# swarth100/dynfu

Measured on AMD Instinct MI355X. Metric: frames/sec (warp-solve + TSDF fuse), 512^3 vol / 2k nodes / VGA depth, higher is better.
Workload: dtype f32; 1 GPU; C2: 512^3 TSDF, 640x480 depth, 2048 nodes, k=4, 262144 vertices, 5 GN x PCG<=256 (tol 1e-6), reference-parity energy (energy.t), lambda=200; parallelism=replicas x1 (one sequence per GPU, no collective), ranks_seen=1, repeats=5

## Files before the change

dynfu_amd/csrc/capi_solver.cpp:

```cpp
#include <algorithm>
#include <cmath>
#include <cstdlib>
#include <cstring>
#include <new>

#include "capi_internal.hpp"
#include "dev_switch.hpp"
#include "solve.hpp"

using namespace dfa::capi;

struct dfa_solver {
    int max_D, max_N, k;
    size_t max_R;
    int ell_cap;
    int asm_resident = 0;
    dfa::SolveView v;
    dfa::SolveState* state;
    double* cost_partials;
    unsigned int* ticket;
    dfa::PlanArena mem;
    GridScratch grid;
    bool has_problem;
    bool timing;
// ... 92 lines not shown
        const size_t areas = (size_t)3 * dfa::solve_team_pcg_rounds();
        mem.alloc(&s->v.team_ctl, 1, true);
        mem.alloc(&s->v.team_mt, areas * s->v.team_stride, true);
        mem.alloc(&s->v.team_words, dfa::solve_team_pcg_words(), true);
        s->team.host_abort = mem.pinned<int>(1);
        if ((rc = plan_status(mem)) == DFA_OK && !s->team.host_abort) rc = fail(DFA_ERR_HIP, "hipHostMalloc (team PCG abort count)");
        if (rc == DFA_OK) {
            s->team.ctl = s->v.team_ctl;
            if (const char* e0 = dfa::dev_env("DFA_MB_TEAM_EPOCH")) s->team.epoch = (unsigned)std::strtoul(e0, nullptr, 0);
        }
    }
    if (rc == DFA_OK) {
        mem.alloc(&s->state, 1);
        mem.alloc(&s->iters_total, 1, true);
        s->host_flag = mem.pinned<int>(4);
        mem.alloc(&s->cost_partials, std::max<size_t>((R + 255) / 256 + 1, 1024) + 1024);
        mem.alloc(&s->ticket, 64, true);
        rc = plan_status(mem);
    }
    if (rc != DFA_OK) {
        dfa_solver_destroy(s);
        return rc;
    }
    *out = s;
    return DFA_OK;
}

void dfa_solver_destroy(dfa_solver* s) {
    if (!s) return;
    s->grid.release();
    s->mb_graphs.release();
// ... 84 lines not shown
                HIP_TRY(hipMemcpyAsync(&s->host_flag[1], &s->state->converged, sizeof(int), hipMemcpyDeviceToHost, st));
                HIP_TRY(hipStreamSynchronize(st));
            }
            if (s->host_flag && s->host_flag[1]) {
                ++not_launched;
                continue;
            }
            ++gn_in_outer;
            if (gn > 0 && p->gn_tol == 0.f && p->lambda > 0.f && !no_regradient) {
                const int ev = bracket_open(s, st);
                HIP_TRY(dfa::solve_regradient(v, s->state, st));
                if (int rc = run_pcg(ev)) return rc;
                continue;
            }
            const bool with_huber = gn == 0 && outer == p->num_iter - 1;
            HIP_TRY(dfa::solve_linearise(v, s->state, s->cost_partials, s->ticket, gn == 0, gn == 0 ? 0 : 1,
                                         p->gn_tol, p->tukey_offset, p->psi_data, w_reg_sq, with_huber ? p->psi_reg : 0.f, nullptr, st));
            huber_done |= with_huber;
            const int ev = bracket_open(s, st);
            HIP_TRY(dfa::solve_assemble(v, s->state, gn == 0 && p->nonlinear_iter > 1, w_reg_sq, s->asm_resident, st));
            if (int rc = run_pcg(ev)) return rc;
        }
    }
    if (s->overlap_fn && gn_launched == 0) s->overlap_fn(s->overlap_user, stream, -1);
    if (not_launched) HIP_TRY(dfa::solve_count_noop(s->state, not_launched, st));
    const bool no_weights = p->num_iter == 0 || p->nonlinear_iter == 0;
    if (!huber_done) HIP_TRY(dfa::solve_huber(v, p->psi_reg, st));
    HIP_TRY(dfa::solve_linearise(v, s->state, s->cost_partials, s->ticket, no_weights ? 1 : 0, 2, 0.f,
                                 p->tukey_offset, p->psi_data, w_reg_sq, 0.f, s->timing ? s->iters_total : nullptr, st));
    return DFA_OK;
}

int dfa_solver_set_overlap_callback(dfa_solver* s, dfa_overlap_fn fn, void* user) {
    REQUIRE(s, "null plan");
    s->overlap_fn = fn, s->overlap_user = user;
    return DFA_OK;
}

const float* dfa_solver_translations(const dfa_solver* s) { return s ? s->v.t : nullptr; }
const float* dfa_solver_node_dq(const dfa_solver* s) { return s ? s->v.node_dq_out : nullptr; }
const float* dfa_solver_tukey_weights(const dfa_solver* s) { return s ? s->v.rtau : nullptr; }
const float* dfa_solver_huber_weights(const dfa_solver* s) { return s ? s->v.huber : nullptr; }
const int32_t* dfa_solver_data_graph(const dfa_solver* s) { return s ? s->v.ridx : nullptr; }
const int32_t* dfa_solver_reg_graph(const dfa_solver* s) { return s ? s->v.reg_idx : nullptr; }
// ... 86 lines not shown
```

dynfu_amd/csrc/solve.hpp:

```cpp
#pragma once
#include <hip/hip_runtime.h>
#include <stdint.h>

#include "kernels.hpp"

namespace dfa {

struct SolveState {
    double initial_cost;
    double cost;
    double final_cost;
    double grad_first;
    int have_initial;
    int done;
    int gn_iters;
    int pcg_iters;
    int max_row_nnz;
    int overflow;
    int pcg_fallback;
    int split_iters;
    unsigned int split_ticket;
    int mb_done;
    int converged;
    int mb_skip, mb_iters;
    int weights_fresh;
    int gn_noop;
    int cost_stale;
    float mb_rz0, mb_gamma_prev[2], mb_alpha_prev[2];
    float amax;
    long long prof[8];
};

__host__ __device__ inline bool solve_rec_ids16(int k) { return k % 8 == 0; }
__host__ __device__ inline int solve_rec_words(int k) { return solve_rec_ids16(k) ? k + k / 2 + 4 : 2 * k + 4; }
__host__ __device__ inline int solve_rec_tail(int k) { return solve_rec_words(k) - 4; }

__device__ __forceinline__ void solve_mark_at_floor(SolveState* st) {
    if (st->weights_fresh) st->converged = 1;
    else if (!st->converged) st->converged = 2;
}

struct TeamCtl {
    unsigned int count[3];
    unsigned int abort[3];
    unsigned int finished[3];
// ... 36 lines not shown
    unsigned long long* team_words;
    int team_stride;
    float* t;
    float* huber;
    float* node_dq_out;
};

constexpr int SOLVE_TG_BLOCKS = 256;
hipError_t solve_build_graph(const SolveView& s, SolveState* state, unsigned int* ticket, int nticket, hipStream_t st);
bool solve_graph_rows_fits(const SolveView& s);
hipError_t solve_build_graph_rows(const SolveView& s, const KnnGridView& grid, SolveState* state, unsigned int* ticket,
                                  int nticket, hipStream_t st);
hipError_t solve_transpose_graph(const int32_t* ridx, size_t total, int D, int32_t* blk_hist, int32_t* node_ptr,
                                 uint32_t* node_list, hipStream_t st);
int solve_residual_blocks(const SolveView& s);
hipError_t solve_linearise(const SolveView& s, SolveState* state, double* cost_partials, unsigned int* ticket,
                           int update_weights, int mode, float gn_tol, float tukey_offset, float psi_data,
                           float w_reg_sq, float huber_psi ,
                           long long* iters_total , hipStream_t st);
hipError_t solve_huber(const SolveView& s, float psi_reg, hipStream_t st);
hipError_t solve_reset(const SolveView& s, SolveState* state, unsigned int* ticket, int nticket, hipStream_t st);
hipError_t solve_assemble(const SolveView& s, SolveState* state, int save_base , float w_reg_sq,
                          int resident_blocks, hipStream_t st);
int solve_assemble_resident_blocks(int k);
hipError_t solve_regradient(const SolveView& s, SolveState* state, hipStream_t st);
int solve_pcg_max_nodes();
__host__ __device__ inline int solve_mb_rows_per_block() { return 16; }
__host__ __device__ inline int solve_mb_blocks(int D) { return (D + 15) / 16; }
struct MbGraphCache {
    struct Entry {
        int it0 = 0, it1 = 0;
        float tol = 0.f;
        SolveView view;
        const SolveState* state = nullptr;
        hipGraphExec_t exec = nullptr;
    };
    Entry e[24];
    int used = 0;
// ... 26 lines not shown
```

dynfu_amd/csrc/solve_assemble.hip:

```cpp
#include <hip/hip_runtime.h>

#include <algorithm>

#include "dev_switch.hpp"
#include "device_math.hpp"
#include "solve.hpp"
#include "solve_internal.hpp"
#include "solve_rows.hpp"

namespace dfa {


constexpr int HASH      = 512;
constexpr int HASH_MASK = HASH - 1;

struct FixedScale {
    float up;
    double down;
};
__device__ __forceinline__ FixedScale solve_fixed_scale(float amax) {
    int e = 0;
    (void)frexpf(fmaxf(amax, 1e-30f), &e);
    e = e < -80 ? -80 : e > 100 ? 100 : e;
    FixedScale f;
// ... 8 lines not shown
}
__device__ __forceinline__ void fixed_add(long long* cell, float v, float up) {
    const float x  = truncf(fabsf(v) * up);
    const float hf = floorf(x * 2.3283064365386963e-10f);
    const uint32_t hi = (uint32_t)hf, lo = (uint32_t)fmaf(hf, -4294967296.f, x);
    atomicAdd(reinterpret_cast<unsigned long long*>(v < 0.f ? cell + HASH : cell), ((unsigned long long)hi << 32) | lo);
}

#ifdef DFA_PCG_PROFILE
__device__ unsigned long long asm_tbuf[32768 * 8];
extern "C" __attribute__((visibility("default"))) int dfa_dev_asm_timing(unsigned long long* out, int n) {
    return (int)hipMemcpyFromSymbol(out, HIP_SYMBOL(asm_tbuf), sizeof(unsigned long long) * 8 * (size_t)n);
}
#endif

template <int K>
__device__ __forceinline__ void assemble_entry(int a, int slot, const int (&idx)[K], const float (&w)[K], float4 et, float up, int* key,
                                               long long* val, int* ovf, float& gx, float& gy, float& gz, float& dsum) {
    float wa = 0.f;
#pragma unroll
    for (int j = 0; j < K; ++j) wa = (j == slot) ? w[j] : wa;
    const float tw = et.w * wa;
    gx += tw * et.x, gy += tw * et.y, gz += tw * et.z;
    if (et.w == 0.f) return;
    uint32_t h0[K];
    int k0[K];
#pragma unroll
    for (int j = 0; j < K; ++j) {
        h0[j] = ((uint32_t)idx[j] * 2654435761u) >> (32 - 9);
        k0[j] = key[h0[j]];
// ... 19 lines not shown
            if (cur == b) {
                fixed_add(&val[h], v, up);
                break;
            }
            if (probes >= HASH) {
                *ovf = 1;
                break;
            }
            h   = (h + 1) & HASH_MASK;
            cur = key[h];
        }
    }
}

template <int K, int T>
__global__ __launch_bounds__(256) void assemble_kernel(SolveView s, SolveState* __restrict__ st, int save_base, float amax_unset) {
    __shared__ int key[HASH];
    __shared__ long long val[2 * HASH];
    __shared__ float gpart[4][3];
    __shared__ int wave_cnt[4];
    __shared__ int ovf;
    if (st->done || st->converged) return;
    const int a = blockIdx.x;
    const int wave = threadIdx.x >> 6, lane = threadIdx.x & 63;
#ifdef DFA_PCG_PROFILE
    long long t0_ = clock64(), t1_, t2_, t3_, t4_;
    const unsigned long long w0_ = wall_clock64();
#endif
    const int beg = s.node_ptr[a], end = s.node_ptr[a + 1];
    const float amax_st = st->amax;
    [[maybe_unused]] uint32_t ent[T];
    if constexpr (T > 1) {
#pragma unroll
        for (int t = 0; t < T; ++t) ent[t] = s.node_list[max(min(beg + 256 * t + (int)threadIdx.x, end - 1), 0)];
    }
    for (int i = threadIdx.x; i < HASH; i += 256) key[i] = -1, val[i] = val[i + HASH] = 0ll;
    if (threadIdx.x == 0) ovf = 0;
    __syncthreads();
#ifdef DFA_PCG_PROFILE
    t1_ = clock64();
#endif

    const FixedScale fx = fixed_scale_for_rows(solve_fixed_scale(amax_st > 0.f ? amax_st : amax_unset), end - beg);
    float gx = 0.f, gy = 0.f, gz = 0.f, dsum = 0.f;
    if constexpr (T > 1) {
        SolveView sk = s;
        sk.k         = K;
        for (int base = beg + (int)threadIdx.x; base - (int)threadIdx.x < end; base += 256 * T) {
            if (base - (int)threadIdx.x != beg) {
#pragma unroll
                for (int t = 0; t < T; ++t) ent[t] = s.node_list[min(base + 256 * t, end - 1)];
            }
            int slot[T], idx[T][K];
// ... 93 lines not shown
        if (total > *(volatile int*)&st->max_row_nnz) atomicMax(&st->max_row_nnz, total);
        if (total > s.ell_cap || ovf) st->overflow = 1;
#ifdef DFA_PCG_PROFILE
        t4_ = clock64();
        if (a == 7 && !s.team_ctl) st->prof[6] = (t1_ - t0_) * 1000000 + (t2_ - t1_), st->prof[7] = (t3_ - t2_) * 1000000 + (t4_ - t3_);
        if (a < 32768) {
            unsigned long long* o = asm_tbuf + 8 * (size_t)a;
            o[0] = w0_, o[1] = wall_clock64() - w0_, o[2] = (unsigned long long)(end - beg), o[3] = (unsigned long long)total;
            o[4] = t1_ - t0_, o[5] = t2_ - t1_, o[6] = t3_ - t2_, o[7] = t4_ - t3_;
        }
#endif
    }
}

template <int K>
__global__ __launch_bounds__(256) void assemble_det_kernel(SolveView s, SolveState* __restrict__ st, int save_base, float amax_unset) {
    __shared__ int key[HASH];
    __shared__ long long val[2 * HASH];
    __shared__ float gpart[4][3], dpart[4];
    __shared__ int ovf, nkeys;
    if (st->done || st->converged) return;
    const int a    = blockIdx.x;
    const int wave = threadIdx.x >> 6, lane = threadIdx.x & 63;
    for (int i = threadIdx.x; i < HASH; i += 256) key[i] = -1, val[i] = val[i + HASH] = 0ll;
    if (threadIdx.x == 0) ovf = 0, nkeys = 0;
    __syncthreads();
    const int beg = s.node_ptr[a], end = s.node_ptr[a + 1];
    const FixedScale fx = fixed_scale_for_rows(solve_fixed_scale(st->amax > 0.f ? st->amax : amax_unset), end - beg);
    float gx = 0.f, gy = 0.f, gz = 0.f, dsum = 0.f;
    for (int p = beg + (int)threadIdx.x; p < end; p += 256) {
        const uint32_t e = s.node_list[p];
        const size_t r   = e / (uint32_t)s.k;
        const int slot   = (int)(e - (uint32_t)r * (uint32_t)s.k);
        int idx[K];
        float w[K];
        const float4 et = load_record<K>(s, r, idx, w);
        float wa = 0.f;
#pragma unroll
        for (int j = 0; j < K; ++j) wa = (j == slot) ? w[j] : wa;
        const float tw = et.w * wa;
        gx += tw * et.x, gy += tw * et.y, gz += tw * et.z;
        if (et.w != 0.f) {
#pragma unroll
// ... 91 lines not shown
    if (asm_chunk(K) == 1) return 0;
    int dev = 0, cus = 0, per_cu = 0;
    if (hipGetDevice(&dev) != hipSuccess || hipDeviceGetAttribute(&cus, hipDeviceAttributeMultiprocessorCount, dev) != hipSuccess ||
        hipOccupancyMaxActiveBlocksPerMultiprocessor(&per_cu, assemble_kernel<K, asm_chunk(K)>, 256, 0) != hipSuccess) {
        (void)hipGetLastError();
        return 0;
    }
    return cus * per_cu;
}

int solve_assemble_resident_blocks(int k) {
    return k <= 4 ? resident_blocks_of<4>() : k <= 8 ? resident_blocks_of<8>() : resident_blocks_of<16>();
}

template <int K>
static void launch_assemble(const SolveView& s, SolveState* state, int save_base, float amax_unset, bool in_flight, hipStream_t st) {
    if (asm_chunk(K) > 1 && in_flight && s.k == K) assemble_kernel<K, asm_chunk(K)><<<s.D, 256, 0, st>>>(s, state, save_base, amax_unset);
    else assemble_kernel<K, 1><<<s.D, 256, 0, st>>>(s, state, save_base, amax_unset);
}

hipError_t solve_assemble(const SolveView& s, SolveState* state, int save_base, float w_reg_sq, int resident_blocks, hipStream_t st) {
    const float amax_unset = std::max(1.0f, w_reg_sq);
    if (s.deterministic) KDISPATCH(assemble_det_kernel, s.k, <<<s.D, 256, 0, st>>>(s, state, save_base, amax_unset));
    else {
        bool in_flight  = s.D <= resident_blocks;
        const int force = dev_env_int("DFA_ASM_IN_FLIGHT", -1);
        if (force >= 0) in_flight = force != 0;
        if (s.k <= 4) launch_assemble<4>(s, state, save_base, amax_unset, in_flight, st);
        else if (s.k <= 8) launch_assemble<8>(s, state, save_base, amax_unset, in_flight, st);
        else launch_assemble<16>(s, state, save_base, amax_unset, in_flight, st);
    }
    return hipGetLastError();
}

}
```

dynfu_amd/csrc/solve_internal.hpp:

```cpp
#pragma once
#include <hip/hip_runtime.h>

#include "device_math.hpp"
#include "kernels.hpp"
#include "solve.hpp"

namespace dfa {

template <int NWAVES>
__device__ __forceinline__ double block_sum(float v, float* red) {
    const float w = wave_total(v);
    if ((threadIdx.x & 63) == 0) red[threadIdx.x >> 6] = w;
    __syncthreads();
    double tot = 0.0;
#pragma unroll
    for (int i = 0; i < NWAVES; ++i) tot += (double)red[i];
    return tot;
}

#ifdef DFA_PCG_PROFILE
#define PROF_MARK(i)                      \
    do {                                  \
        const long long now_ = clock64(); \
        pc_[i] += now_ - last_;           \
// ... 9 lines not shown
    if ((threadIdx.x & 63) == 0) red[threadIdx.x >> 6] = w;
    __syncthreads();
    float tot = 0.f;
#pragma unroll
    for (int i = 0; i < NWAVES; ++i) tot += red[i];
    return tot;
}

#define KDISPATCH(kernel, k, ...)                      \
    do {                                               \
        if ((k) <= 4) kernel<4> __VA_ARGS__;           \
        else if ((k) <= 8) kernel<8> __VA_ARGS__;      \
        else kernel<16> __VA_ARGS__;                   \
    } while (0)

template <class Kernel>
static hipError_t allow_big_lds(Kernel* k) {
    return allow_dynamic_lds((const void*)k, 160 * 1024 - 1024);
}

#pragma GCC visibility push(hidden)
hipError_t launch_mb_pcg(const SolveView& s, SolveState* state, int max_iter, float pcg_tol, int* host_flag,
                         MbGraphCache* gc, hipStream_t st);
hipError_t launch_team_pcg(const SolveView& s, SolveState* state, int max_iter, float pcg_tol, TeamPcg* tp, hipStream_t st);
#pragma GCC visibility pop

}
```

dynfu_amd/csrc/solve_linearise.hip:

```cpp
#include <hip/hip_runtime.h>

#include "dev_switch.hpp"
#include "dq_device.hpp"
#include "solve.hpp"
#include "solve_internal.hpp"
#include "solve_rows.hpp"

namespace dfa {


template <int K>
__device__ __forceinline__ float tukey_weight_of(const SolveView& s, const int (&n)[K], const float (&w)[K], f3 c, f3 l, float tukey_offset,
                                                 float psi_data) {
    DQ sum = dq_identity();
#pragma unroll
    for (int h = 0; h < K; h += 4) {
        float tx[4], ty[4], tz[4];
        DQ q[4];
#pragma unroll
        for (int jj = 0; jj < 4; ++jj) {
            const int nn = n[h + jj] >= 0 ? n[h + jj] : 0;
            tx[jj] = s.t[3 * nn], ty[jj] = s.t[3 * nn + 1], tz[jj] = s.t[3 * nn + 2];
            q[jj]  = dq_load(s.node_dq + 8 * (size_t)nn);
        }
#pragma unroll
        for (int jj = 0; jj < 4; ++jj) {
            if (n[h + jj] >= 0) {
                const DQ cur = dq_mul(dq_from_translation(tx[jj], ty[jj], tz[jj]), q[jj]);
                sum          = dq_mul(sum, dq_scale(cur, w[h + jj]));
            }
        }
    }
    const f3 warped = dq_transform(dq_normalize(sum), c);
    const float ex = l.x - warped.x, ey = l.y - warped.y, ez = l.z - warped.z;
    const float d = sqrtf(ex * ex + ey * ey + ez * ez) / tukey_offset;
    if (d < psi_data) {
        const double q = 1.0 - ((double)d * (double)d) / ((double)psi_data * (double)psi_data);
        return (float)(q * q);
    }
    return 0.f;
}
template <int K>
__device__ __forceinline__ float tukey_weight(const SolveView& s, size_t v, float tukey_offset, float psi_data) {
    const f3 c = mk3(s.canon[3 * v], s.canon[3 * v + 1], s.canon[3 * v + 2]);
    int n[K];
    float w[K];
    load_row_graph<K>(s, v, n, w);
    const f3 l = mk3(s.live[3 * v], s.live[3 * v + 1], s.live[3 * v + 2]);
    return tukey_weight_of<K>(s, n, w, c, l, tukey_offset, psi_data);
}

__device__ __forceinline__ void huber_node(const SolveView& s, int i, float psi_reg) {
    const DQ dq_i = dq_mul(dq_from_translation(s.t[3 * i], s.t[3 * i + 1], s.t[3 * i + 2]),
                           dq_load(s.node_dq + 8 * (size_t)i));
    float h = 0.f;
    for (int j = 0; j < s.k; ++j) {
        const int m = s.reg_idx[(size_t)i * s.k + j];
        if (m < 0) break;
        const f3 pm   = mk3(s.node_pos[3 * m], s.node_pos[3 * m + 1], s.node_pos[3 * m + 2]);
        const DQ dq_m = dq_mul(dq_from_translation(s.t[3 * m], s.t[3 * m + 1], s.t[3 * m + 2]),
                               dq_load(s.node_dq + 8 * (size_t)m));
        const f3 pa = dq_transform(dq_i, pm), pb = dq_transform(dq_m, pm);
        const float ex = pa.x - pb.x, ey = pa.y - pb.y, ez = pa.z - pb.z;
        const float err = sqrtf(ex * ex + ey * ey + ez * ez);
        h               = fabsf(err) <= psi_reg ? 1.f : psi_reg / fabsf(err);
    }
    s.huber[i] = h;
}
__global__ __launch_bounds__(256) void huber_kernel(SolveView s, float psi_reg) {
    const int i = blockIdx.x * blockDim.x + threadIdx.x;
    if (i < s.D) huber_node(s, i, psi_reg);
}

struct LineariseArgs {
    int update_weights;
    int mode;
    float gn_tol, tukey_offset, psi_data, w_reg_sq;
    long long* iters_total;
    float huber_psi;
};

constexpr int LIN_SHARDS     = 32;
constexpr int LIN_MAX_BLOCKS = 1024;

template <int K>
struct LinRow {
    int n[K];
    float w[K];
    float bx, by, bz, tau;
    f3 c, l;
};
template <int K>
__device__ __forceinline__ void lin_row_load(const SolveView& s, size_t r, int update_weights, LinRow<K>& q) {
    load_row_graph<K>(s, r, q.n, q.w);
    q.bx = s.rb[3 * r], q.by = s.rb[3 * r + 1], q.bz = s.rb[3 * r + 2];
    q.tau = 0.f, q.c = q.l = mk3(0.f, 0.f, 0.f);
    if (!update_weights) q.tau = s.rtau[r];
    else if (r < (size_t)s.N) {
        q.c = mk3(s.canon[3 * r], s.canon[3 * r + 1], s.canon[3 * r + 2]);
        q.l = mk3(s.live[3 * r], s.live[3 * r + 1], s.live[3 * r + 2]);
    }
}
template <int K>
__device__ __forceinline__ void lin_row_finish(const SolveView& s, size_t r, const LineariseArgs& a, const LinRow<K>& q, double& c, float& amax) {
    float tau = q.tau;
    if (a.update_weights) {
        tau       = r < (size_t)s.N ? tukey_weight_of<K>(s, q.n, q.w, q.c, q.l, a.tukey_offset, a.psi_data) : a.w_reg_sq;
        s.rtau[r] = tau;
    }
    float sx = 0.f, sy = 0.f, sz = 0.f;
    float tx[K], ty[K], tz[K];
#pragma unroll
    for (int j = 0; j < K; ++j) {
        const int nn = q.n[j] >= 0 ? q.n[j] : 0;
        tx[j] = s.t[3 * nn], ty[j] = s.t[3 * nn + 1], tz[j] = s.t[3 * nn + 2];
    }
    float wm = 0.f;
#pragma unroll
    for (int j = 0; j < K; ++j)
        if (q.n[j] >= 0) sx += q.w[j] * tx[j], sy += q.w[j] * ty[j], sz += q.w[j] * tz[j], wm = fmaxf(wm, fabsf(q.w[j]));
    amax = fmaxf(amax, tau * wm * wm);
    const float ex = q.bx - sx, ey = q.by - sy, ez = q.bz - sz;
    *(float4*)(s.re + r * (size_t)solve_rec_words(s.k) + solve_rec_tail(s.k)) = make_float4(ex, ey, ez, tau);
    c += (double)tau * ((double)ex * ex + (double)ey * ey + (double)ez * ez);
}

template <int K, bool TWO>
__global__ __launch_bounds__(256) void linearise_kernel(SolveView s, SolveState* __restrict__ st,
                                                        double* __restrict__ cost_partials,
                                                        unsigned int* __restrict__ ticket ,
                                                        LineariseArgs a) {
    __shared__ double wsum[4];
    __shared__ int is_last;
    if (a.huber_psi > 0.f)
        for (int i = blockIdx.x * blockDim.x + threadIdx.x; i < s.D; i += gridDim.x * blockDim.x) huber_node(s, i, a.huber_psi);
    if (a.mode == 2) {
        for (int i = blockIdx.x * blockDim.x + threadIdx.x; i < s.D; i += gridDim.x * blockDim.x) {
            const DQ out = dq_mul(dq_from_translation(s.t[3 * i], s.t[3 * i + 1], s.t[3 * i + 2]),
                                  dq_load(s.node_dq + 8 * (size_t)i));
            dq_store(s.node_dq_out + 8 * (size_t)i, out);
        }
        if (blockIdx.x == 0 && threadIdx.x == 0 && a.iters_total) *a.iters_total += st->pcg_iters;
    }
    if (st->converged == 1 || (st->converged && !a.update_weights)) {
        if (a.mode != 2 || (st->have_initial && !st->cost_stale)) return;
    }
    const size_t R = (size_t)s.N + (size_t)s.D * s.k;
    double c       = 0.0;
    float amax     = 0.f;
    const size_t stride = (size_t)gridDim.x * blockDim.x;
    size_t r_first      = (size_t)blockIdx.x * blockDim.x + threadIdx.x;
    if constexpr (TWO) {
        if (r_first < R) {
            const size_t r1 = r_first + stride;
            LinRow<K> q0, q1;
            lin_row_load<K>(s, r_first, a.update_weights, q0);
            if (r1 < R) lin_row_load<K>(s, r1, a.update_weights, q1);
            lin_row_finish<K>(s, r_first, a, q0, c, amax);
            if (r1 < R) lin_row_finish<K>(s, r1, a, q1, c, amax);
            r_first = r1 + stride;
        }
    }
    for (size_t r = r_first; r < R; r += stride) {
        float tau;
        if (a.update_weights) {
            tau       = r < (size_t)s.N ? tukey_weight<K>(s, r, a.tukey_offset, a.psi_data) : a.w_reg_sq;
            s.rtau[r] = tau;
        } else {
            tau = s.rtau[r];
        }
        float sx = 0.f, sy = 0.f, sz = 0.f;
        {
            int n[K];
            float w[K], tx[K], ty[K], tz[K];
            load_row_graph<K>(s, r, n, w);
#pragma unroll
            for (int j = 0; j < K; ++j) {
                const int nn = n[j] >= 0 ? n[j] : 0;
                tx[j] = s.t[3 * nn], ty[j] = s.t[3 * nn + 1], tz[j] = s.t[3 * nn + 2];
            }
            float wm = 0.f;
#pragma unroll
            for (int j = 0; j < K; ++j)
                if (n[j] >= 0) sx += w[j] * tx[j], sy += w[j] * ty[j], sz += w[j] * tz[j], wm = fmaxf(wm, fabsf(w[j]));
            amax = fmaxf(amax, tau * wm * wm);
        }
        const float ex = s.rb[3 * r] - sx, ey = s.rb[3 * r + 1] - sy, ez = s.rb[3 * r + 2] - sz;
        *(float4*)(s.re + r * (size_t)solve_rec_words(s.k) + solve_rec_tail(s.k)) = make_float4(ex, ey, ez, tau);
        c += (double)tau * ((double)ex * ex + (double)ey * ey + (double)ez * ez);
    }
    c = wave_sum_all(c);
    __shared__ float wmax[4];
#pragma unroll
    for (int o = 32; o > 0; o >>= 1) amax = fmaxf(amax, __shfl_xor(amax, o, 64));
    if ((threadIdx.x & 63) == 0) wsum[threadIdx.x >> 6] = c, wmax[threadIdx.x >> 6] = amax;
    __syncthreads();
    if (threadIdx.x == 0) {
        __hip_atomic_store(&cost_partials[blockIdx.x], (wsum[0] + wsum[1]) + (wsum[2] + wsum[3]), __ATOMIC_RELAXED,
                           __HIP_MEMORY_SCOPE_AGENT);
        if (a.update_weights)
            __hip_atomic_store(&cost_partials[LIN_MAX_BLOCKS + blockIdx.x], (double)fmaxf(fmaxf(wmax[0], wmax[1]), fmaxf(wmax[2], wmax[3])),
                               __ATOMIC_RELAXED, __HIP_MEMORY_SCOPE_AGENT);
        asm volatile("s_waitcnt vmcnt(0)" ::: "memory");
        const unsigned int shard   = blockIdx.x % LIN_SHARDS;
        const unsigned int members = (gridDim.x - shard + LIN_SHARDS - 1) / LIN_SHARDS;
        const unsigned int nshards = min((unsigned int)LIN_SHARDS, gridDim.x);
        int last                   = 0;
        if (__hip_atomic_fetch_add(&ticket[shard], 1u, __ATOMIC_RELAXED, __HIP_MEMORY_SCOPE_AGENT) == members - 1) {
            __hip_atomic_store(&ticket[shard], 0u, __ATOMIC_RELAXED, __HIP_MEMORY_SCOPE_AGENT);
            if (__hip_atomic_fetch_add(&ticket[LIN_SHARDS], 1u, __ATOMIC_RELAXED, __HIP_MEMORY_SCOPE_AGENT) ==
                nshards - 1) {
                __hip_atomic_store(&ticket[LIN_SHARDS], 0u, __ATOMIC_RELAXED, __HIP_MEMORY_SCOPE_AGENT);
                last = 1;
            }
        }
        is_last = last;
    }
    __syncthreads();
    if (!is_last) return;

    __shared__ double sm[256];
    __shared__ double smx[256];
    double acc = 0.0, mx = 0.0;
    {
        constexpr int Q = LIN_MAX_BLOCKS / 256;
        double cq[Q], mq[Q];
#pragma unroll
        for (int q = 0; q < Q; ++q) {
            const unsigned int i = min(threadIdx.x + 256u * q, gridDim.x - 1);
            cq[q] = __hip_atomic_load(&cost_partials[i], __ATOMIC_RELAXED, __HIP_MEMORY_SCOPE_AGENT);
            mq[q] = a.update_weights ? __hip_atomic_load(&cost_partials[LIN_MAX_BLOCKS + i], __ATOMIC_RELAXED, __HIP_MEMORY_SCOPE_AGENT) : 0.0;
        }
#pragma unroll
        for (int q = 0; q < Q; ++q)
            if (threadIdx.x + 256u * q < gridDim.x) acc += cq[q], mx = fmax(mx, mq[q]);
    }
    sm[threadIdx.x] = acc, smx[threadIdx.x] = mx;
    __syncthreads();
    for (int o = 128; o > 0; o >>= 1) {
        if ((int)threadIdx.x < o) sm[threadIdx.x] += sm[threadIdx.x + o], smx[threadIdx.x] = fmax(smx[threadIdx.x], smx[threadIdx.x + o]);
        __syncthreads();
    }
    if (threadIdx.x == 0) {
        const double cost = sm[0];
        if (a.update_weights) st->amax = (float)smx[0];
        if (!st->have_initial) st->initial_cost = cost, st->have_initial = 1;
        if (a.mode == 0) st->done = 0;
        if (a.mode == 1 && !st->done && a.gn_tol > 0.f && (st->cost - cost) <= (double)a.gn_tol * st->cost)
            st->done = 1;
        st->cost       = cost;
        st->final_cost = cost;
        st->cost_stale = 0;
        if (a.mode != 2) st->weights_fresh = a.update_weights;
        if (a.mode != 2 && a.update_weights && st->converged == 2) st->converged = 0;
    }
}


int solve_residual_blocks(const SolveView& s) {
    const size_t R  = (size_t)s.N + (size_t)s.D * s.k;
    const size_t nb = (R + 255) / 256;
    return (int)(nb < (size_t)LIN_MAX_BLOCKS ? nb : (size_t)LIN_MAX_BLOCKS);
}

constexpr bool lin_two_rows(int K) { return K == 4; }

template <int K>
static void launch_linearise(const SolveView& s, SolveState* state, double* cost_partials, unsigned int* ticket, const LineariseArgs& a,
                             int nb, hipStream_t st) {
#ifdef DFA_DEV_AB
    if (dev_env_int("DFA_LIN_TWO_ROWS", lin_two_rows(K)) != 0) linearise_kernel<K, true><<<nb, 256, 0, st>>>(s, state, cost_partials, ticket, a);
    else linearise_kernel<K, false><<<nb, 256, 0, st>>>(s, state, cost_partials, ticket, a);
#else
    linearise_kernel<K, lin_two_rows(K)><<<nb, 256, 0, st>>>(s, state, cost_partials, ticket, a);
#endif
}

hipError_t solve_linearise(const SolveView& s, SolveState* state, double* cost_partials, unsigned int* ticket,
                           int update_weights, int mode, float gn_tol, float tukey_offset, float psi_data,
                           float w_reg_sq, float huber_psi, long long* iters_total, hipStream_t st) {
    const int nb = solve_residual_blocks(s);
    LineariseArgs a{update_weights, mode, gn_tol, tukey_offset, psi_data, w_reg_sq, iters_total, huber_psi};
    if (s.k <= 4) launch_linearise<4>(s, state, cost_partials, ticket, a, nb, st);
    else if (s.k <= 8) launch_linearise<8>(s, state, cost_partials, ticket, a, nb, st);
    else launch_linearise<16>(s, state, cost_partials, ticket, a, nb, st);
    return hipGetLastError();
}

hipError_t solve_huber(const SolveView& s, float psi_reg, hipStream_t st) {
    huber_kernel<<<(s.D + 255) / 256, 256, 0, st>>>(s, psi_reg);
    return hipGetLastError();
}

__global__ __launch_bounds__(256) void regradient_kernel(SolveView s, SolveState* __restrict__ st) {
    if (st->done || st->converged) return;
    const int a = blockIdx.x * blockDim.x + threadIdx.x;
    if (a == 0) st->cost_stale = 1, st->weights_fresh = 0;
// ... 20 lines not shown
```

Before: 1697 frames/s.

## Hand off linearise cost reduction to assemble kernel, skipping last-block ticket

On the first Gauss-Newton step, when weights are updated and there is no tolerance check, the linearise kernel now writes its per-block cost and max partials without atomics and returns, skipping the last-block ticket and final reduction. The assemble kernel gets one extra block that performs the cost reduction and bookkeeping. Every assemble block rebuilds amax directly from the float partials using a DPP wave max, rather than reading it from the state. The aim is to take the serialized tail reduction and the atomics off the critical path, at the cost of redundant amax loads in each assemble block and a more complex state handoff. The row code is also refactored to share its weighted sums with the Tukey weight computation.

```diff
diff --git a/dynfu_amd/csrc/capi_solver.cpp b/dynfu_amd/csrc/capi_solver.cpp
--- a/dynfu_amd/csrc/capi_solver.cpp
+++ b/dynfu_amd/csrc/capi_solver.cpp
@@ -130,7 +130,7 @@
         mem.alloc(&s->state, 1);
         mem.alloc(&s->iters_total, 1, true);
         s->host_flag = mem.pinned<int>(4);
-        mem.alloc(&s->cost_partials, std::max<size_t>((R + 255) / 256 + 1, 1024) + 1024);
+        mem.alloc(&s->cost_partials, dfa::solve_cost_partials_len());
         mem.alloc(&s->ticket, 64, true);
         rc = plan_status(mem);
     }
@@ -245,11 +245,13 @@
                 continue;
             }
             const bool with_huber = gn == 0 && outer == p->num_iter - 1;
-            HIP_TRY(dfa::solve_linearise(v, s->state, s->cost_partials, s->ticket, gn == 0, gn == 0 ? 0 : 1,
-                                         p->gn_tol, p->tukey_offset, p->psi_data, w_reg_sq, with_huber ? p->psi_reg : 0.f, nullptr, st));
+            const bool handoff = dfa::solve_lin_handoff(gn == 0, gn == 0 ? 0 : 1, p->gn_tol) && dfa::dev_env_int("DFA_LIN_HANDOFF", 1) != 0;
+            HIP_TRY(dfa::solve_linearise(v, s->state, s->cost_partials, s->ticket, gn == 0, gn == 0 ? 0 : 1, p->gn_tol,
+                                         p->tukey_offset, p->psi_data, w_reg_sq, with_huber ? p->psi_reg : 0.f, nullptr, handoff, st));
             huber_done |= with_huber;
             const int ev = bracket_open(s, st);
-            HIP_TRY(dfa::solve_assemble(v, s->state, gn == 0 && p->nonlinear_iter > 1, w_reg_sq, s->asm_resident, st));
+            HIP_TRY(dfa::solve_assemble(v, s->state, gn == 0 && p->nonlinear_iter > 1, w_reg_sq, s->asm_resident,
+                                        handoff ? s->cost_partials : nullptr, st));
             if (int rc = run_pcg(ev)) return rc;
         }
     }
@@ -258,7 +260,7 @@
     const bool no_weights = p->num_iter == 0 || p->nonlinear_iter == 0;
     if (!huber_done) HIP_TRY(dfa::solve_huber(v, p->psi_reg, st));
     HIP_TRY(dfa::solve_linearise(v, s->state, s->cost_partials, s->ticket, no_weights ? 1 : 0, 2, 0.f,
-                                 p->tukey_offset, p->psi_data, w_reg_sq, 0.f, s->timing ? s->iters_total : nullptr, st));
+                                 p->tukey_offset, p->psi_data, w_reg_sq, 0.f, s->timing ? s->iters_total : nullptr, false, st));
     return DFA_OK;
 }
 
diff --git a/dynfu_amd/csrc/solve.hpp b/dynfu_amd/csrc/solve.hpp
--- a/dynfu_amd/csrc/solve.hpp
+++ b/dynfu_amd/csrc/solve.hpp
@@ -29,6 +29,7 @@
     float mb_rz0, mb_gamma_prev[2], mb_alpha_prev[2];
     float amax;
     long long prof[8];
+    int lin_pending;
 };
 
 __host__ __device__ inline bool solve_rec_ids16(int k) { return k % 8 == 0; }
@@ -95,14 +96,17 @@
 hipError_t solve_transpose_graph(const int32_t* ridx, size_t total, int D, int32_t* blk_hist, int32_t* node_ptr,
                                  uint32_t* node_list, hipStream_t st);
 int solve_residual_blocks(const SolveView& s);
+size_t solve_cost_partials_len();
 hipError_t solve_linearise(const SolveView& s, SolveState* state, double* cost_partials, unsigned int* ticket,
                            int update_weights, int mode, float gn_tol, float tukey_offset, float psi_data,
                            float w_reg_sq, float huber_psi ,
-                           long long* iters_total , hipStream_t st);
+                           long long* iters_total , bool handoff,
+                           hipStream_t st);
+inline bool solve_lin_handoff(int update_weights, int mode, float gn_tol) { return update_weights == 1 && mode == 0 && gn_tol == 0.f; }
 hipError_t solve_huber(const SolveView& s, float psi_reg, hipStream_t st);
 hipError_t solve_reset(const SolveView& s, SolveState* state, unsigned int* ticket, int nticket, hipStream_t st);
 hipError_t solve_assemble(const SolveView& s, SolveState* state, int save_base , float w_reg_sq,
-                          int resident_blocks, hipStream_t st);
+                          int resident_blocks, const double* handoff_partials, hipStream_t st);
 int solve_assemble_resident_blocks(int k);
 hipError_t solve_regradient(const SolveView& s, SolveState* state, hipStream_t st);
 int solve_pcg_max_nodes();
diff --git a/dynfu_amd/csrc/solve_assemble.hip b/dynfu_amd/csrc/solve_assemble.hip
--- a/dynfu_amd/csrc/solve_assemble.hip
+++ b/dynfu_amd/csrc/solve_assemble.hip
@@ -46,6 +46,34 @@
 }
 #endif
 
+__device__ __forceinline__ float amax_partials_load(const double* cost_partials, int nb) {
+    static_assert(LIN_MAX_BLOCKS == 4 * 256, "one float4 per thread of a 256-thread workgroup");
+    const float4 m = reinterpret_cast<const float4*>(lin_max_floats(cost_partials))[threadIdx.x];
+    const int i    = 4 * (int)threadIdx.x;
+    return fmaxf(fmaxf(i < nb ? m.x : 0.f, i + 1 < nb ? m.y : 0.f), fmaxf(i + 2 < nb ? m.z : 0.f, i + 3 < nb ? m.w : 0.f));
+}
+template <int CTRL, int ROW_MASK>
+__device__ __forceinline__ float dpp_max0(float v) {
+    return fmaxf(v, __int_as_float(__builtin_amdgcn_update_dpp(0, __float_as_int(v), CTRL, ROW_MASK, 0xf, false)));
+}
+__device__ __forceinline__ void amax_partials_publish(float am, float* amax_w ) {
+    am = dpp_max0<0x111, 0xf>(am), am = dpp_max0<0x112, 0xf>(am), am = dpp_max0<0x114, 0xf>(am), am = dpp_max0<0x118, 0xf>(am);
+    am = dpp_max0<0x142, 0xa>(am), am = dpp_max0<0x143, 0xc>(am);
+    const float wave_max = __int_as_float(__builtin_amdgcn_readlane(__float_as_int(am), 63));
+    amax_w[__builtin_amdgcn_readfirstlane(threadIdx.x) >> 6] = wave_max;
+}
+__device__ __forceinline__ float amax_partials_collect(const float* amax_w) {
+    return __int_as_float(__builtin_amdgcn_readfirstlane(__float_as_int(fmaxf(fmaxf(amax_w[0], amax_w[1]), fmaxf(amax_w[2], amax_w[3])))));
+}
+__device__ __forceinline__ void assemble_book_cost(SolveState* st, const double* cost_partials, int nb, double* sm, double* smx) {
+    if (!st->lin_pending) return;
+    lin_sum_partials<false>(cost_partials, (unsigned int)nb, true, sm, smx);
+    if (threadIdx.x == 0) {
+        lin_book_cost(st, sm[0], smx[0], 1, 0, 0.f, false);
+        st->lin_pending = 0;
+    }
+}
+
 template <int K>
 __device__ __forceinline__ void assemble_entry(int a, int slot, const int (&idx)[K], const float (&w)[K], float4 et, float up, int* key,
                                                long long* val, int* ovf, float& gx, float& gy, float& gz, float& dsum) {
@@ -95,12 +123,18 @@
 }
 
 template <int K, int T>
-__global__ __launch_bounds__(256) void assemble_kernel(SolveView s, SolveState* __restrict__ st, int save_base, float amax_unset) {
+__global__ __launch_bounds__(256) void assemble_kernel(SolveView s, SolveState* __restrict__ st, int save_base, float amax_unset,
+                                                       const double* __restrict__ cost_partials ) {
     __shared__ int key[HASH];
     __shared__ long long val[2 * HASH];
     __shared__ float gpart[4][3];
+    __shared__ float amax_w[4];
     __shared__ int wave_cnt[4];
     __shared__ int ovf;
+    if ((int)blockIdx.x == s.D) {
+        assemble_book_cost(st, cost_partials, lin_blocks(s.N, s.D, s.k), reinterpret_cast<double*>(val), reinterpret_cast<double*>(val) + 256);
+        return;
+    }
     if (st->done || st->converged) return;
     const int a = blockIdx.x;
     const int wave = threadIdx.x >> 6, lane = threadIdx.x & 63;
@@ -109,15 +143,17 @@
     const unsigned long long w0_ = wall_clock64();
 #endif
     const int beg = s.node_ptr[a], end = s.node_ptr[a + 1];
-    const float amax_st = st->amax;
     [[maybe_unused]] uint32_t ent[T];
     if constexpr (T > 1) {
 #pragma unroll
         for (int t = 0; t < T; ++t) ent[t] = s.node_list[max(min(beg + 256 * t + (int)threadIdx.x, end - 1), 0)];
     }
+    float amax_st = cost_partials ? amax_partials_load(cost_partials, lin_blocks(s.N, s.D, s.k)) : st->amax;
     for (int i = threadIdx.x; i < HASH; i += 256) key[i] = -1, val[i] = val[i + HASH] = 0ll;
     if (threadIdx.x == 0) ovf = 0;
-    __syncthreads();
+    if (cost_partials) amax_partials_publish(amax_st, amax_w);
+    __syncthreads();
+    if (cost_partials) amax_st = amax_partials_collect(amax_w);
 #ifdef DFA_PCG_PROFILE
     t1_ = clock64();
 #endif
@@ -241,19 +277,27 @@
 }
 
 template <int K>
-__global__ __launch_bounds__(256) void assemble_det_kernel(SolveView s, SolveState* __restrict__ st, int save_base, float amax_unset) {
+__global__ __launch_bounds__(256) void assemble_det_kernel(SolveView s, SolveState* __restrict__ st, int save_base, float amax_unset,
+                                                           const double* __restrict__ cost_partials ) {
     __shared__ int key[HASH];
     __shared__ long long val[2 * HASH];
-    __shared__ float gpart[4][3], dpart[4];
+    __shared__ float gpart[4][3], dpart[4], amax_w[4];
     __shared__ int ovf, nkeys;
+    if ((int)blockIdx.x == s.D) {
+        assemble_book_cost(st, cost_partials, lin_blocks(s.N, s.D, s.k), reinterpret_cast<double*>(val), reinterpret_cast<double*>(val) + 256);
+        return;
+    }
     if (st->done || st->converged) return;
     const int a    = blockIdx.x;
     const int wave = threadIdx.x >> 6, lane = threadIdx.x & 63;
+    float amax_st  = cost_partials ? amax_partials_load(cost_partials, lin_blocks(s.N, s.D, s.k)) : st->amax;
     for (int i = threadIdx.x; i < HASH; i += 256) key[i] = -1, val[i] = val[i + HASH] = 0ll;
     if (threadIdx.x == 0) ovf = 0, nkeys = 0;
-    __syncthreads();
+    if (cost_partials) amax_partials_publish(amax_st, amax_w);
+    __syncthreads();
+    if (cost_partials) amax_st = amax_partials_collect(amax_w);
     const int beg = s.node_ptr[a], end = s.node_ptr[a + 1];
-    const FixedScale fx = fixed_scale_for_rows(solve_fixed_scale(st->amax > 0.f ? st->amax : amax_unset), end - beg);
+    const FixedScale fx = fixed_scale_for_rows(solve_fixed_scale(amax_st > 0.f ? amax_st : amax_unset), end - beg);
     float gx = 0.f, gy = 0.f, gz = 0.f, dsum = 0.f;
     for (int p = beg + (int)threadIdx.x; p < end; p += 256) {
         const uint32_t e = s.node_list[p];
@@ -375,21 +419,25 @@
 }
 
 template <int K>
-static void launch_assemble(const SolveView& s, SolveState* state, int save_base, float amax_unset, bool in_flight, hipStream_t st) {
-    if (asm_chunk(K) > 1 && in_flight && s.k == K) assemble_kernel<K, asm_chunk(K)><<<s.D, 256, 0, st>>>(s, state, save_base, amax_unset);
-    else assemble_kernel<K, 1><<<s.D, 256, 0, st>>>(s, state, save_base, amax_unset);
-}
-
-hipError_t solve_assemble(const SolveView& s, SolveState* state, int save_base, float w_reg_sq, int resident_blocks, hipStream_t st) {
+static void launch_assemble(const SolveView& s, SolveState* state, int save_base, float amax_unset, bool in_flight, const double* partials,
+                            int nb, hipStream_t st) {
+    const int grid = s.D + (nb > 0 ? 1 : 0);
+    if (asm_chunk(K) > 1 && in_flight && s.k == K) assemble_kernel<K, asm_chunk(K)><<<grid, 256, 0, st>>>(s, state, save_base, amax_unset, partials);
+    else assemble_kernel<K, 1><<<grid, 256, 0, st>>>(s, state, save_base, amax_unset, partials);
+}
+
+hipError_t solve_assemble(const SolveView& s, SolveState* state, int save_base, float w_reg_sq, int resident_blocks,
+                          const double* handoff_partials, hipStream_t st) {
     const float amax_unset = std::max(1.0f, w_reg_sq);
-    if (s.deterministic) KDISPATCH(assemble_det_kernel, s.k, <<<s.D, 256, 0, st>>>(s, state, save_base, amax_unset));
+    const int nb           = handoff_partials ? solve_residual_blocks(s) : 0;
+    if (s.deterministic) KDISPATCH(assemble_det_kernel, s.k, <<<s.D + (nb > 0 ? 1 : 0), 256, 0, st>>>(s, state, save_base, amax_unset, handoff_partials));
     else {
         bool in_flight  = s.D <= resident_blocks;
         const int force = dev_env_int("DFA_ASM_IN_FLIGHT", -1);
         if (force >= 0) in_flight = force != 0;
-        if (s.k <= 4) launch_assemble<4>(s, state, save_base, amax_unset, in_flight, st);
-        else if (s.k <= 8) launch_assemble<8>(s, state, save_base, amax_unset, in_flight, st);
-        else launch_assemble<16>(s, state, save_base, amax_unset, in_flight, st);
+        if (s.k <= 4) launch_assemble<4>(s, state, save_base, amax_unset, in_flight, handoff_partials, nb, st);
+        else if (s.k <= 8) launch_assemble<8>(s, state, save_base, amax_unset, in_flight, handoff_partials, nb, st);
+        else launch_assemble<16>(s, state, save_base, amax_unset, in_flight, handoff_partials, nb, st);
     }
     return hipGetLastError();
 }
diff --git a/dynfu_amd/csrc/solve_internal.hpp b/dynfu_amd/csrc/solve_internal.hpp
--- a/dynfu_amd/csrc/solve_internal.hpp
+++ b/dynfu_amd/csrc/solve_internal.hpp
@@ -47,6 +47,60 @@
         else kernel<16> __VA_ARGS__;                   \
     } while (0)
 
+constexpr int LIN_SHARDS     = 32;
+constexpr int LIN_MAX_BLOCKS = 1024;
+constexpr size_t LIN_PARTIALS_LEN = 2 * LIN_MAX_BLOCKS + LIN_MAX_BLOCKS / 2;
+__host__ __device__ inline float* lin_max_floats(double* cost_partials) { return reinterpret_cast<float*>(cost_partials + 2 * LIN_MAX_BLOCKS); }
+__host__ __device__ inline const float* lin_max_floats(const double* cost_partials) {
+    return reinterpret_cast<const float*>(cost_partials + 2 * LIN_MAX_BLOCKS);
+}
+__host__ __device__ inline int lin_blocks(int N, int D, int k) {
+    const size_t R  = (size_t)N + (size_t)D * k;
+    const size_t nb = (R + 255) / 256;
+    return (int)(nb < (size_t)LIN_MAX_BLOCKS ? nb : (size_t)LIN_MAX_BLOCKS);
+}
+
+template <bool SAME_LAUNCH>
+__device__ __forceinline__ void lin_sum_partials(const double* cost_partials, unsigned int nb, bool with_max, double* sm ,
+                                                 double* smx ) {
+    double acc = 0.0, mx = 0.0;
+    constexpr int Q = LIN_MAX_BLOCKS / 256;
+    double cq[Q], mq[Q];
+#pragma unroll
+    for (int q = 0; q < Q; ++q) {
+        const unsigned int i = min(threadIdx.x + 256u * q, nb - 1);
+        if constexpr (SAME_LAUNCH) {
+            cq[q] = __hip_atomic_load(&cost_partials[i], __ATOMIC_RELAXED, __HIP_MEMORY_SCOPE_AGENT);
+            mq[q] = with_max ? __hip_atomic_load(&cost_partials[LIN_MAX_BLOCKS + i], __ATOMIC_RELAXED, __HIP_MEMORY_SCOPE_AGENT) : 0.0;
+        } else {
+            cq[q] = cost_partials[i];
+            mq[q] = with_max ? cost_partials[LIN_MAX_BLOCKS + i] : 0.0;
+        }
+    }
+#pragma unroll
+    for (int q = 0; q < Q; ++q)
+        if (threadIdx.x + 256u * q < nb) acc += cq[q], mx = fmax(mx, mq[q]);
+    sm[threadIdx.x] = acc, smx[threadIdx.x] = mx;
+    __syncthreads();
+    for (int o = 128; o > 0; o >>= 1) {
+        if ((int)threadIdx.x < o) sm[threadIdx.x] += sm[threadIdx.x + o], smx[threadIdx.x] = fmax(smx[threadIdx.x], smx[threadIdx.x + o]);
+        __syncthreads();
+    }
+}
+
+__device__ __forceinline__ void lin_book_cost(SolveState* st, double cost, double amax, int update_weights, int mode, float gn_tol,
+                                              bool clear_outer) {
+    if (update_weights) st->amax = (float)amax;
+    if (!st->have_initial) st->initial_cost = cost, st->have_initial = 1;
+    if (mode == 0) st->done = 0;
+    if (mode == 1 && !st->done && gn_tol > 0.f && (st->cost - cost) <= (double)gn_tol * st->cost) st->done = 1;
+    st->cost       = cost;
+    st->final_cost = cost;
+    st->cost_stale = 0;
+    if (mode != 2) st->weights_fresh = update_weights;
+    if (clear_outer && mode != 2 && update_weights && st->converged == 2) st->converged = 0;
+}
+
 template <class Kernel>
 static hipError_t allow_big_lds(Kernel* k) {
     return allow_dynamic_lds((const void*)k, 160 * 1024 - 1024);
diff --git a/dynfu_amd/csrc/solve_linearise.hip b/dynfu_amd/csrc/solve_linearise.hip
--- a/dynfu_amd/csrc/solve_linearise.hip
+++ b/dynfu_amd/csrc/solve_linearise.hip
@@ -9,9 +9,17 @@
 namespace dfa {
 
 
-template <int K>
+struct RowSums {
+    float sx = 0.f, sy = 0.f, sz = 0.f, wm = 0.f;
+    __device__ __forceinline__ void add(float w, float tx, float ty, float tz) {
+        sx += w * tx, sy += w * ty, sz += w * tz, wm = fmaxf(wm, fabsf(w));
+    }
+};
+
+template <int K, bool B_AHEAD>
 __device__ __forceinline__ float tukey_weight_of(const SolveView& s, const int (&n)[K], const float (&w)[K], f3 c, f3 l, float tukey_offset,
-                                                 float psi_data) {
+                                                 float psi_data, f3 b, f3& e, float& wm) {
+    RowSums rs;
     DQ sum = dq_identity();
 #pragma unroll
     for (int h = 0; h < K; h += 4) {
@@ -23,6 +31,10 @@
             tx[jj] = s.t[3 * nn], ty[jj] = s.t[3 * nn + 1], tz[jj] = s.t[3 * nn + 2];
             q[jj]  = dq_load(s.node_dq + 8 * (size_t)nn);
         }
+#pragma unroll
+        for (int jj = 0; jj < 4; ++jj)
+            if (n[h + jj] >= 0) rs.add(w[h + jj], tx[jj], ty[jj], tz[jj]);
+        if (h + 4 >= K) e = B_AHEAD ? mk3(b.x - rs.sx, b.y - rs.sy, b.z - rs.sz) : mk3(rs.sx, rs.sy, rs.sz), wm = rs.wm;
 #pragma unroll
         for (int jj = 0; jj < 4; ++jj) {
             if (n[h + jj] >= 0) {
@@ -40,16 +52,6 @@
     }
     return 0.f;
 }
-template <int K>
-__device__ __forceinline__ float tukey_weight(const SolveView& s, size_t v, float tukey_offset, float psi_data) {
-    const f3 c = mk3(s.canon[3 * v], s.canon[3 * v + 1], s.canon[3 * v + 2]);
-    int n[K];
-    float w[K];
-    load_row_graph<K>(s, v, n, w);
-    const f3 l = mk3(s.live[3 * v], s.live[3 * v + 1], s.live[3 * v + 2]);
-    return tukey_weight_of<K>(s, n, w, c, l, tukey_offset, psi_data);
-}
-
 __device__ __forceinline__ void huber_node(const SolveView& s, int i, float psi_reg) {
     const DQ dq_i = dq_mul(dq_from_translation(s.t[3 * i], s.t[3 * i + 1], s.t[3 * i + 2]),
                            dq_load(s.node_dq + 8 * (size_t)i));
@@ -77,11 +79,28 @@
     int mode;
     float gn_tol, tukey_offset, psi_data, w_reg_sq;
     long long* iters_total;
+    int handoff;
     float huber_psi;
 };
 
-constexpr int LIN_SHARDS     = 32;
-constexpr int LIN_MAX_BLOCKS = 1024;
+#ifdef DFA_PCG_PROFILE
+__device__ unsigned long long lin_tbuf[1024 * 8];
+extern "C" __attribute__((visibility("default"))) int dfa_dev_lin_timing(unsigned long long* out, int n) {
+    return (int)hipMemcpyFromSymbol(out, HIP_SYMBOL(lin_tbuf), sizeof(unsigned long long) * 8 * (size_t)n);
+}
+#define LIN_MARK(i) (lw_[i] = wall_clock64())
+#define LIN_MARKS_OUT(last)                                                          \
+    do {                                                                             \
+        if (threadIdx.x == 0 && a.mode != 2) {                                       \
+            lw_[3 + 3 * (last)] = wall_clock64(), lw_[7] = (last);                   \
+            if (last) lw_[3] = lw_[6];                                               \
+            for (int i_ = 0; i_ < 8; ++i_) lin_tbuf[8 * blockIdx.x + i_] = lw_[i_];  \
+        }                                                                            \
+    } while (0)
+#else
+#define LIN_MARK(i)
+#define LIN_MARKS_OUT(last)
+#endif
 
 template <int K>
 struct LinRow {
@@ -90,10 +109,11 @@
     float bx, by, bz, tau;
     f3 c, l;
 };
-template <int K>
+template <int K, bool WITH_B>
 __device__ __forceinline__ void lin_row_load(const SolveView& s, size_t r, int update_weights, LinRow<K>& q) {
     load_row_graph<K>(s, r, q.n, q.w);
-    q.bx = s.rb[3 * r], q.by = s.rb[3 * r + 1], q.bz = s.rb[3 * r + 2];
+    q.bx = q.by = q.bz = 0.f;
+    if (WITH_B) q.bx = s.rb[3 * r], q.by = s.rb[3 * r + 1], q.bz = s.rb[3 * r + 2];
     q.tau = 0.f, q.c = q.l = mk3(0.f, 0.f, 0.f);
     if (!update_weights) q.tau = s.rtau[r];
     else if (r < (size_t)s.N) {
@@ -101,28 +121,57 @@
         q.l = mk3(s.live[3 * r], s.live[3 * r + 1], s.live[3 * r + 2]);
     }
 }
+template <int K, bool B_AHEAD>
+__device__ __forceinline__ void lin_row_sums(const SolveView& s, const int (&n)[K], const float (&w)[K], f3 b, f3& e, float& wm) {
+    float tx[K], ty[K], tz[K];
+#pragma unroll
+    for (int j = 0; j < K; ++j) {
+        const int nn = n[j] >= 0 ? n[j] : 0;
+        tx[j] = s.t[3 * nn], ty[j] = s.t[3 * nn + 1], tz[j] = s.t[3 * nn + 2];
+    }
+    RowSums rs;
+#pragma unroll
+    for (int j = 0; j < K; ++j)
+        if (n[j] >= 0) rs.add(w[j], tx[j], ty[j], tz[j]);
+    e = B_AHEAD ? mk3(b.x - rs.sx, b.y - rs.sy, b.z - rs.sz) : mk3(rs.sx, rs.sy, rs.sz), wm = rs.wm;
+}
+__device__ __forceinline__ void lin_row_store(const SolveView& s, size_t r, f3 e, float tau, float wm, double& c, float& amax) {
+    amax = fmaxf(amax, tau * wm * wm);
+    *(float4*)(s.re + r * (size_t)solve_rec_words(s.k) + solve_rec_tail(s.k)) = make_float4(e.x, e.y, e.z, tau);
+    c += (double)tau * ((double)e.x * e.x + (double)e.y * e.y + (double)e.z * e.z);
+}
+template <int K, bool WITH_B>
+__device__ __forceinline__ void lin_row_finish(const SolveView& s, size_t r, const LineariseArgs& a, const LinRow<K>& q, double& c, float& amax) {
+    float tau = q.tau, wm;
+    f3 e;
+    const f3 b = WITH_B ? mk3(q.bx, q.by, q.bz) : mk3(s.rb[3 * r], s.rb[3 * r + 1], s.rb[3 * r + 2]);
+    if (a.update_weights && r < (size_t)s.N) tau = tukey_weight_of<K, WITH_B>(s, q.n, q.w, q.c, q.l, a.tukey_offset, a.psi_data, b, e, wm);
+    else {
+        lin_row_sums<K, WITH_B>(s, q.n, q.w, b, e, wm);
+        if (a.update_weights) tau = a.w_reg_sq;
+    }
+    if (a.update_weights) s.rtau[r] = tau;
+    if (!WITH_B) e = mk3(b.x - e.x, b.y - e.y, b.z - e.z);
+    lin_row_store(s, r, e, tau, wm, c, amax);
+}
 template <int K>
-__device__ __forceinline__ void lin_row_finish(const SolveView& s, size_t r, const LineariseArgs& a, const LinRow<K>& q, double& c, float& amax) {
-    float tau = q.tau;
-    if (a.update_weights) {
-        tau       = r < (size_t)s.N ? tukey_weight_of<K>(s, q.n, q.w, q.c, q.l, a.tukey_offset, a.psi_data) : a.w_reg_sq;
-        s.rtau[r] = tau;
-    }
-    float sx = 0.f, sy = 0.f, sz = 0.f;
-    float tx[K], ty[K], tz[K];
-#pragma unroll
-    for (int j = 0; j < K; ++j) {
-        const int nn = q.n[j] >= 0 ? q.n[j] : 0;
-        tx[j] = s.t[3 * nn], ty[j] = s.t[3 * nn + 1], tz[j] = s.t[3 * nn + 2];
-    }
-    float wm = 0.f;
-#pragma unroll
-    for (int j = 0; j < K; ++j)
-        if (q.n[j] >= 0) sx += q.w[j] * tx[j], sy += q.w[j] * ty[j], sz += q.w[j] * tz[j], wm = fmaxf(wm, fabsf(q.w[j]));
-    amax = fmaxf(amax, tau * wm * wm);
-    const float ex = q.bx - sx, ey = q.by - sy, ez = q.bz - sz;
-    *(float4*)(s.re + r * (size_t)solve_rec_words(s.k) + solve_rec_tail(s.k)) = make_float4(ex, ey, ez, tau);
-    c += (double)tau * ((double)ex * ex + (double)ey * ey + (double)ez * ez);
+__device__ __forceinline__ void lin_row_plain(const SolveView& s, size_t r, const LineariseArgs& a, double& c, float& amax) {
+    int n[K];
+    float w[K];
+    load_row_graph<K>(s, r, n, w);
+    float tau, wm;
+    f3 e;
+    if (a.update_weights && r < (size_t)s.N) {
+        const f3 cp = mk3(s.canon[3 * r], s.canon[3 * r + 1], s.canon[3 * r + 2]);
+        const f3 l  = mk3(s.live[3 * r], s.live[3 * r + 1], s.live[3 * r + 2]);
+        tau         = tukey_weight_of<K, false>(s, n, w, cp, l, a.tukey_offset, a.psi_data, mk3(0.f, 0.f, 0.f), e, wm);
+    } else {
+        tau = a.update_weights ? a.w_reg_sq : s.rtau[r];
+        lin_row_sums<K, false>(s, n, w, mk3(0.f, 0.f, 0.f), e, wm);
+    }
+    if (a.update_weights) s.rtau[r] = tau;
+    e = mk3(s.rb[3 * r] - e.x, s.rb[3 * r + 1] - e.y, s.rb[3 * r + 2] - e.z);
+    lin_row_store(s, r, e, tau, wm, c, amax);
 }
 
 template <int K, bool TWO>
@@ -145,6 +194,14 @@
     if (st->converged == 1 || (st->converged && !a.update_weights)) {
         if (a.mode != 2 || (st->have_initial && !st->cost_stale)) return;
     }
+    if (a.handoff && blockIdx.x == 0 && threadIdx.x == 0) {
+        if (st->converged == 2) st->converged = 0;
+        st->lin_pending = 1;
+    }
+#ifdef DFA_PCG_PROFILE
+    unsigned long long lw_[8] = {};
+    LIN_MARK(0);
+#endif
     const size_t R = (size_t)s.N + (size_t)s.D * s.k;
     double c       = 0.0;
     float amax     = 0.f;
@@ -154,40 +211,15 @@
         if (r_first < R) {
             const size_t r1 = r_first + stride;
             LinRow<K> q0, q1;
-            lin_row_load<K>(s, r_first, a.update_weights, q0);
-            if (r1 < R) lin_row_load<K>(s, r1, a.update_weights, q1);
-            lin_row_finish<K>(s, r_first, a, q0, c, amax);
-            if (r1 < R) lin_row_finish<K>(s, r1, a, q1, c, amax);
+            lin_row_load<K, true>(s, r_first, a.update_weights, q0);
+            if (r1 < R) lin_row_load<K, false>(s, r1, a.update_weights, q1);
+            lin_row_finish<K, true>(s, r_first, a, q0, c, amax);
+            if (r1 < R) lin_row_finish<K, false>(s, r1, a, q1, c, amax);
             r_first = r1 + stride;
         }
     }
     for (size_t r = r_first; r < R; r += stride) {
-        float tau;
-        if (a.update_weights) {
-            tau       = r < (size_t)s.N ? tukey_weight<K>(s, r, a.tukey_offset, a.psi_data) : a.w_reg_sq;
-            s.rtau[r] = tau;
-        } else {
-            tau = s.rtau[r];
-        }
-        float sx = 0.f, sy = 0.f, sz = 0.f;
-        {
-            int n[K];
-            float w[K], tx[K], ty[K], tz[K];
-            load_row_graph<K>(s, r, n, w);
-#pragma unroll
-            for (int j = 0; j < K; ++j) {
-                const int nn = n[j] >= 0 ? n[j] : 0;
-                tx[j] = s.t[3 * nn], ty[j] = s.t[3 * nn + 1], tz[j] = s.t[3 * nn + 2];
-            }
-            float wm = 0.f;
-#pragma unroll
-            for (int j = 0; j < K; ++j)
-                if (n[j] >= 0) sx += w[j] * tx[j], sy += w[j] * ty[j], sz += w[j] * tz[j], wm = fmaxf(wm, fabsf(w[j]));
-            amax = fmaxf(amax, tau * wm * wm);
-        }
-        const float ex = s.rb[3 * r] - sx, ey = s.rb[3 * r + 1] - sy, ez = s.rb[3 * r + 2] - sz;
-        *(float4*)(s.re + r * (size_t)solve_rec_words(s.k) + solve_rec_tail(s.k)) = make_float4(ex, ey, ez, tau);
-        c += (double)tau * ((double)ex * ex + (double)ey * ey + (double)ez * ez);
+        lin_row_plain<K>(s, r, a, c, amax);
     }
     c = wave_sum_all(c);
     __shared__ float wmax[4];
@@ -195,6 +227,18 @@
     for (int o = 32; o > 0; o >>= 1) amax = fmaxf(amax, __shfl_xor(amax, o, 64));
     if ((threadIdx.x & 63) == 0) wsum[threadIdx.x >> 6] = c, wmax[threadIdx.x >> 6] = amax;
     __syncthreads();
+    LIN_MARK(1);
+    if (a.handoff) {
+        if (threadIdx.x == 0) {
+            cost_partials[blockIdx.x]                  = (wsum[0] + wsum[1]) + (wsum[2] + wsum[3]);
+            const float mx = fmaxf(fmaxf(wmax[0], wmax[1]), fmaxf(wmax[2], wmax[3]));
+            cost_partials[LIN_MAX_BLOCKS + blockIdx.x] = (double)mx;
+            lin_max_floats(cost_partials)[blockIdx.x]  = mx;
+        }
+        LIN_MARK(2);
+        LIN_MARKS_OUT(0);
+        return;
+    }
     if (threadIdx.x == 0) {
         __hip_atomic_store(&cost_partials[blockIdx.x], (wsum[0] + wsum[1]) + (wsum[2] + wsum[3]), __ATOMIC_RELAXED,
                            __HIP_MEMORY_SCOPE_AGENT);
@@ -217,51 +261,24 @@
         is_last = last;
     }
     __syncthreads();
-    if (!is_last) return;
+    LIN_MARK(2);
+    if (!is_last) {
+        LIN_MARKS_OUT(0);
+        return;
+    }
+    LIN_MARK(4);
 
     __shared__ double sm[256];
     __shared__ double smx[256];
-    double acc = 0.0, mx = 0.0;
-    {
-        constexpr int Q = LIN_MAX_BLOCKS / 256;
-        double cq[Q], mq[Q];
-#pragma unroll
-        for (int q = 0; q < Q; ++q) {
-            const unsigned int i = min(threadIdx.x + 256u * q, gridDim.x - 1);
-            cq[q] = __hip_atomic_load(&cost_partials[i], __ATOMIC_RELAXED, __HIP_MEMORY_SCOPE_AGENT);
-            mq[q] = a.update_weights ? __hip_atomic_load(&cost_partials[LIN_MAX_BLOCKS + i], __ATOMIC_RELAXED, __HIP_MEMORY_SCOPE_AGENT) : 0.0;
-        }
-#pragma unroll
-        for (int q = 0; q < Q; ++q)
-            if (threadIdx.x + 256u * q < gridDim.x) acc += cq[q], mx = fmax(mx, mq[q]);
-    }
-    sm[threadIdx.x] = acc, smx[threadIdx.x] = mx;
-    __syncthreads();
-    for (int o = 128; o > 0; o >>= 1) {
-        if ((int)threadIdx.x < o) sm[threadIdx.x] += sm[threadIdx.x + o], smx[threadIdx.x] = fmax(smx[threadIdx.x], smx[threadIdx.x + o]);
-        __syncthreads();
-    }
-    if (threadIdx.x == 0) {
-        const double cost = sm[0];
-        if (a.update_weights) st->amax = (float)smx[0];
-        if (!st->have_initial) st->initial_cost = cost, st->have_initial = 1;
-        if (a.mode == 0) st->done = 0;
-        if (a.mode == 1 && !st->done && a.gn_tol > 0.f && (st->cost - cost) <= (double)a.gn_tol * st->cost)
-            st->done = 1;
-        st->cost       = cost;
-        st->final_cost = cost;
-        st->cost_stale = 0;
-        if (a.mode != 2) st->weights_fresh = a.update_weights;
-        if (a.mode != 2 && a.update_weights && st->converged == 2) st->converged = 0;
-    }
-}
-
-
-int solve_residual_blocks(const SolveView& s) {
-    const size_t R  = (size_t)s.N + (size_t)s.D * s.k;
-    const size_t nb = (R + 255) / 256;
-    return (int)(nb < (size_t)LIN_MAX_BLOCKS ? nb : (size_t)LIN_MAX_BLOCKS);
-}
+    lin_sum_partials<true>(cost_partials, gridDim.x, a.update_weights != 0, sm, smx);
+    LIN_MARK(5);
+    if (threadIdx.x == 0) lin_book_cost(st, sm[0], smx[0], a.update_weights, a.mode, a.gn_tol, true);
+    LIN_MARKS_OUT(1);
+}
+
+
+int solve_residual_blocks(const SolveView& s) { return lin_blocks(s.N, s.D, s.k); }
+size_t solve_cost_partials_len() { return LIN_PARTIALS_LEN; }
 
 constexpr bool lin_two_rows(int K) { return K == 4; }
 
@@ -278,9 +295,10 @@
 
 hipError_t solve_linearise(const SolveView& s, SolveState* state, double* cost_partials, unsigned int* ticket,
                            int update_weights, int mode, float gn_tol, float tukey_offset, float psi_data,
-                           float w_reg_sq, float huber_psi, long long* iters_total, hipStream_t st) {
+                           float w_reg_sq, float huber_psi, long long* iters_total, bool handoff, hipStream_t st) {
     const int nb = solve_residual_blocks(s);
-    LineariseArgs a{update_weights, mode, gn_tol, tukey_offset, psi_data, w_reg_sq, iters_total, huber_psi};
+    if (handoff && !solve_lin_handoff(update_weights, mode, gn_tol)) return hipErrorInvalidValue;
+    LineariseArgs a{update_weights, mode, gn_tol, tukey_offset, psi_data, w_reg_sq, iters_total, handoff ? 1 : 0, huber_psi};
     if (s.k <= 4) launch_linearise<4>(s, state, cost_partials, ticket, a, nb, st);
     else if (s.k <= 8) launch_linearise<8>(s, state, cost_partials, ticket, a, nb, st);
     else launch_linearise<16>(s, state, cost_partials, ticket, a, nb, st);
```

Result: faster. 1732 frames/s, median of 6 (+2.1%).
